# td-kwj-zp2023/webgpu-msm-twisted-edwards

Measured on AMD Instinct MI355X. Metric: MSMs/sec at n=2^20 Twisted-Edwards BLS12 (pipelined throughput = 1000/ms_per_step; single-MSM latency in latency_ms), higher is better.
Workload: dtype u32

## Files before the change

webgpu-msm-twisted-edwards_amd/csrc/kernels.hip.hpp:

```cpp
#pragma once
#include <hip/hip_runtime.h>
#include "curve.hpp"

namespace te {

#define TE_BATCH_MAX 8
struct batch_ptrs { const uint4* p[TE_BATCH_MAX]; };
struct batch_slabs { uint32_t s[TE_BATCH_MAX]; };

struct digits_params {
  uint32_t half[10];
  uint32_t zero_digit;
  uint32_t sc_stride;
  uint32_t n, nst;
  int num_windows;
  int w_first, w_step, nw_local;
  uint32_t half_code, logS, P, CH, chunk_len;
};

struct pnt_slot { uint4 q[8]; };
__device__ __forceinline__ void prep_points_block(uint32_t blk, uint4* __restrict__ lds, const uint4* __restrict__ pts, pnt_slot* __restrict__ recs, uint32_t n) {
  const uint32_t t = threadIdx.x, base = blk * 256u;
  const bool active = t < 256u;
  const uint32_t pieces_in = (n - base < 256u ? n - base : 256u) * 4u;
// ... 530 lines not shown
  __syncthreads();
  const uint32_t c0 = cnt_s[t];
  const size_t gb = (size_t)k * g.B + (size_t)p * g.S + t;
  if (!single) {
    if (c0) atomicAdd(&a.bucket_count[gb], c0);
    wait_own_accesses();
    __syncthreads();
    if (t == 0) pj[2] = (handoff_arrive(&a.part_ticket[k * g.P + p]) + 1u == (cntp + TE_L2_CAP - 1u) / TE_L2_CAP) ? 1u : 0u;
    __syncthreads();
    if (pj[2]) (void)seg_plan_block(p, k, t < g.S ? ld_agent(a.bucket_count + gb) : 0u, g, a.pa, PL, pb, cntp, sbp);
    return;
  }
  if (t < g.S) a.bucket_count[gb] = c0;
  const uint32_t ex = seg_plan_block(p, k, c0, g, a.pa, PL, pb, cntp, sbp);
  if (t < g.S) a.pa.bucket_cursor[gb] = pb + ex + c0;
  off_s[t] = ex;
  __syncthreads();
#pragma unroll
  for (int c = 0; c < 5; c++) {
    uint32_t kv[8], iv[8]; piece_group<PK>(r, c, kv, iv);
    const uint32_t e0 = ((uint32_t)c * 256u + t) * 8u;
#pragma unroll
    for (int e = 0; e < 8; e++) {
      const uint32_t pos = e0 + (uint32_t)e;
      if (pos >= head && pos < total) list[atomicAdd(&off_s[kv[e] & 0x7fffu], 1u)] = iv[e] | ((kv[e] >> 15) << 31);
    }
  }
  __syncthreads();
  uint32_t* out = a.sorted + (size_t)k * g.n + pb;
  for (uint32_t s = t; s < cntp; s += 256u) out[s] = list[s];
}

#define TE_ORDER_REGS 32u
__device__ __forceinline__ void order_scatter_block(uint32_t ob, uint32_t nob, uint32_t* __restrict__ lds, const uint32_t* __restrict__ lenv, uint32_t ids,
                                                    const uint32_t* __restrict__ size_hist, uint32_t* __restrict__ rel_cursor,
                                                    uint32_t* __restrict__ order, uint32_t* __restrict__ num_segments, uint32_t max_len) {
  uint32_t* const h = lds; uint32_t* const base = lds + 1024; uint32_t* const sm = lds + 2048;
  const uint32_t per = (ids + nob - 1) / nob;
  const uint32_t lo = min(ids, ob * per), hi = min(ids, lo + per);
  const bool in_regs = per <= TE_ORDER_REGS * 256u;
  uint32_t lv[TE_ORDER_REGS];
  if (in_regs) {
#pragma unroll
    for (uint32_t j = 0; j < TE_ORDER_REGS; j++) { const uint32_t g = lo + j * 256u + threadIdx.x; lv[j] = g < hi ? lenv[g] : TE_SEG_INVALID; }
  }
  for (uint32_t j = threadIdx.x; j < 1024u; j += 256u) h[j] = 0;
  {
    uint32_t run = 0;
    for (uint32_t c = (1023u - min(max_len, 1023u)) >> 8; c < 4u; c++) {
      const uint32_t s = 1023u - (c * 256u + threadIdx.x);
      uint32_t part[TE_HIST_COPIES];
#pragma unroll
      for (uint32_t r = 0; r < TE_HIST_COPIES; r++) part[r] = size_hist[r * 1024u + s];
      uint32_t cnt_s = 0;
#pragma unroll
      for (uint32_t r = 0; r < TE_HIST_COPIES; r++) cnt_s += part[r];
      uint32_t bt;
      const uint32_t ex = block_excl_scan(cnt_s, sm, bt);
      base[s] = run + ex;
      run += bt;
    }
    if (ob == 0 && threadIdx.x == 0) *num_segments = run;
  }
  __syncthreads();
  if (in_regs) {
#pragma unroll
    for (uint32_t j = 0; j < TE_ORDER_REGS; j++) if (lv[j] != TE_SEG_INVALID) atomicAdd(&h[min(lv[j], 1023u)], 1u);
  } else {
    for (uint32_t g = lo + threadIdx.x; g < hi; g += 256u) { const uint32_t l = lenv[g]; if (l != TE_SEG_INVALID) atomicAdd(&h[min(l, 1023u)], 1u); }
  }
  __syncthreads();
  for (uint32_t j = threadIdx.x; j < 1024u; j += 256u) { base[j] += h[j] ? atomicAdd(&rel_cursor[j], h[j]) : 0u; h[j] = 0; }
  __syncthreads();
  if (in_regs) {
#pragma unroll
    for (uint32_t j = 0; j < TE_ORDER_REGS; j++) {
      if (lv[j] == TE_SEG_INVALID) continue;
      const uint32_t sz = min(lv[j], 1023u);
      order[base[sz] + atomicAdd(&h[sz], 1u)] = lo + j * 256u + threadIdx.x;
    }
  } else {
    for (uint32_t g = lo + threadIdx.x; g < hi; g += 256u) {
      const uint32_t l = lenv[g];
      if (l == TE_SEG_INVALID) continue;
      const uint32_t sz = min(l, 1023u);
      order[base[sz] + atomicAdd(&h[sz], 1u)] = g;
    }
  }
}

#define TE_PLACE_LDS_WORDS (4u * 256u + TE_L2_LIST + TE_L2_LIST / 4u + 2u + 17u)
template <bool PK>
__device__ __forceinline__ void l2_place_piece(uint32_t p, uint32_t k, uint32_t a0, uint32_t b0, uint32_t* __restrict__ lds,
                                               const uint16_t* __restrict__ part_keys, const uint32_t* __restrict__ part_idx,
                                               uint32_t* __restrict__ bucket_cursor, uint32_t* __restrict__ sorted, const sort_geom& g) {
  uint32_t* const cnt_s = lds; uint32_t* const lex_s = lds + 256; uint32_t* const off_s = lds + 512; uint32_t* const gbase_s = lds + 768;
  uint32_t* const list = lds + 1024;
  uint8_t* const list_b = reinterpret_cast<uint8_t*>(list + TE_L2_LIST);
  uint32_t* const sm = list + TE_L2_LIST + TE_L2_LIST / 4u + 2u;
  const uint32_t t = threadIdx.x, len = b0 - a0;
  const uint16_t* keys_row = part_keys + (size_t)k * g.nst; const uint32_t* idx_row = part_idx + (size_t)k * g.nst;
  uint32_t* out = sorted + (size_t)k * g.n;
  cnt_s[t] = 0u;
  __syncthreads();
  piece_regs r; uint32_t head, total;
  load_piece<PK>(keys_row, idx_row, a0, b0, t, true, r, head, total);
#pragma unroll
  for (int c = 0; c < 5; c++) {
    uint32_t kv[8], iv[8]; piece_group<PK>(r, c, kv, iv);
    const uint32_t e0 = ((uint32_t)c * 256u + t) * 8u;
#pragma unroll
    for (int e = 0; e < 8; e++) { const uint32_t pos = e0 + (uint32_t)e; if (pos >= head && pos < total) atomicAdd(&cnt_s[kv[e] & 0x7fffu], 1u); }
  }
  __syncthreads();
  wave0_excl_scan(cnt_s, lex_s, 256u, &sm[16]);
  {
    const uint32_t c0 = cnt_s[t];
    gbase_s[t] = c0 ? atomicAdd(&bucket_cursor[(size_t)k * g.B + (size_t)p * g.S + t], c0) : 0u;
  }
  __syncthreads();
  off_s[t] = lex_s[t];
  gbase_s[t] -= lex_s[t];
  __syncthreads();
#pragma unroll
  for (int c = 0; c < 5; c++) {
    uint32_t kv[8], iv[8]; piece_group<PK>(r, c, kv, iv);
    const uint32_t e0 = ((uint32_t)c * 256u + t) * 8u;
#pragma unroll
    for (int e = 0; e < 8; e++) {
      const uint32_t pos = e0 + (uint32_t)e;
      if (pos >= head && pos < total) {
        const uint32_t b = kv[e] & 0x7fffu;
        const uint32_t slot = atomicAdd(&off_s[b], 1u);
        list[slot] = iv[e] | ((kv[e] >> 15) << 31); list_b[slot] = (uint8_t)b;
      }
    }
  }
  __syncthreads();
  for (uint32_t s = t; s < len; s += 256u) out[gbase_s[list_b[s]] + s] = list[s];
}

struct order_args { const uint32_t* lenv; uint32_t ids; const uint32_t* size_hist; uint32_t* rel_cursor; uint32_t* order; uint32_t* num_segments; uint32_t order_cols, max_len; };
template <bool PK>
__global__ void __launch_bounds__(256, TE_L2_WAVES) k_l2_place_order(const uint16_t* __restrict__ part_keys, const uint32_t* __restrict__ part_idx,
                                                           const uint32_t* __restrict__ part_start, const uint32_t* __restrict__ part_count,
                                                           uint32_t* __restrict__ bucket_cursor, uint32_t* __restrict__ sorted, sort_geom g, order_args oa) {
  __shared__ uint32_t lds[TE_PLACE_LDS_WORDS];
  if (blockIdx.x < oa.order_cols) {
    order_scatter_block(blockIdx.y * oa.order_cols + blockIdx.x, gridDim.y * oa.order_cols, lds, oa.lenv, oa.ids, oa.size_hist, oa.rel_cursor, oa.order, oa.num_segments, oa.max_len);
    return;
  }
  const uint32_t k = gridDim.y - 1u - blockIdx.y;
  const uint32_t px = blockIdx.x - oa.order_cols, extra = gridDim.x - oa.order_cols - g.P, bx = px < extra ? g.P + px : px - extra;
  const uint32_t* pc = part_count + k * g.P;
  uint32_t p, j;
  if (!l2_piece_of_block(bx, pc, g.P, bx < g.P ? 0u : part_count[gridDim.y * g.P + k], lds, lds + 32, p, j)) return;
  const uint32_t cntp = pc[p], pb = part_start[k * g.P + p];
  if (cntp <= TE_L2_CAP) return;
  const uint32_t a0 = pb + j * TE_L2_CAP;
  l2_place_piece<PK>(p, k, a0, min(pb + cntp, a0 + TE_L2_CAP), lds, part_keys, part_idx, bucket_cursor, sorted, g);
}

template <int N> struct geo {
  static constexpr uint32_t PW = 4u * N;
  static constexpr uint32_t PQ = PW / 4u;
  static constexpr uint32_t RW = N == 9 ? 27u : 4u * N;
  static constexpr uint32_t SQ = N == 9 ? 8u : N;
  static constexpr uint32_t LQ = (RW + 3u) / 4u;
};
template <int N> struct rec_slot { uint4 q[geo<N>::SQ]; };
static_assert(sizeof(rec_slot<9>) == sizeof(pnt_slot) && sizeof(rec_slot<14>) == 224, "record slots");

template <int N> __device__ __forceinline__ pnt_t<N> load_pnt(const rec_slot<N>* __restrict__ recs, uint32_t entry) {
  const uint4* q = recs[entry & 0x7fffffffu].q;
  constexpr uint32_t LQ = geo<N>::LQ;
  uint4 u[LQ];
#pragma unroll
  for (uint32_t j = 0; j < LQ; j++) u[j] = q[j];
  uint32_t w[4 * LQ];
#pragma unroll
  for (uint32_t j = 0; j < LQ; j++) { w[4 * j] = u[j].x; w[4 * j + 1] = u[j].y; w[4 * j + 2] = u[j].z; w[4 * j + 3] = u[j].w; }
  pnt_t<N> r;
// ... 50 lines not shown
  uint32_t w[42];
#pragma unroll
  for (int j = 0; j < 10; j++) { w[4 * j] = u[j].v[0]; w[4 * j + 1] = u[j].v[1]; w[4 * j + 2] = u[j].v[2]; w[4 * j + 3] = u[j].v[3]; }
  w[40] = t.v[0]; w[41] = t.v[1];
  pnt_aff377 r;
#pragma unroll
  for (int j = 0; j < 14; j++) { r.hm.v[j] = w[j]; r.hp.v[j] = w[14 + j]; r.dt.v[j] = w[28 + j]; }
  return r;
}
__device__ __forceinline__ void store_pnt_aff377(rec_aff377* dst, const pnt_aff377& r) {
#pragma unroll
  for (int j = 0; j < 14; j++) { dst->w[j] = r.hm.v[j]; dst->w[14 + j] = r.hp.v[j]; dst->w[28 + j] = r.dt.v[j]; }
}
template <int N, int RK> struct rec_kind;
template <int N> struct rec_kind<N, 0> {
  using slot = rec_slot<N>; using pnt = pnt_t<N>;
  static __device__ __forceinline__ pnt load(const slot* __restrict__ recs, uint32_t e) { return load_pnt<N>(recs, e); }
};
template <> struct rec_kind<14, 1> {
  using slot = rec_aff377; using pnt = pnt_aff377;
  static __device__ __forceinline__ pnt load(const slot* __restrict__ recs, uint32_t e) { return load_pnt_aff377(recs, e); }
};

struct __attribute__((aligned(4))) idx4 { uint32_t v[4]; };
#define TE_CLK_SLOTS 64u
#define TE_IDX_STRIP 16u
template <int N, int RK = 0>
__global__ void __launch_bounds__(256, N == 9 ? 3 : 2) k_accumulate(const typename rec_kind<N, RK>::slot* __restrict__ recs, const uint32_t* __restrict__ sorted,
                                                    const uint32_t* __restrict__ bucket_start, const uint32_t* __restrict__ bucket_count,
                                                    const uint32_t* __restrict__ seg_base, const uint32_t* __restrict__ seg_bucket,
                                                    const uint32_t* __restrict__ seg_lenv, const uint32_t* __restrict__ order,
                                                    const uint32_t* __restrict__ num_segments, ete_t<N>* __restrict__ buckets,
                                                    ete_t<N>* __restrict__ seg_out, uint32_t n, uint32_t logB, uint32_t seg_len, uint32_t ids, uint32_t onto,
                                                    uint32_t win_per_msm, batch_slabs slabs, unsigned long long* __restrict__ clk) {
  __shared__ uint32_t idx_strip[256 * TE_IDX_STRIP];
  using RT = rec_kind<N, RK>; using P = typename RT::pnt;
#if defined(TE_ACC_TWO_WAVES)
  if constexpr (N == 9) asm volatile("" ::: "v175");
#endif
  unsigned long long* const slot = clk ? clk + (blockIdx.x & (TE_CLK_SLOTS - 1u)) : nullptr;
  const unsigned long long t0_wall = clk ? (unsigned long long)wall_clock64() : 0ull, t0_core = clk ? (unsigned long long)clock64() : 0ull;
  if (clk && threadIdx.x == 0) atomicMax(slot, ~t0_wall);
  const uint32_t gid = blockIdx.x * 256u + threadIdx.x;
  if (gid >= (order ? *num_segments : ids)) return;
  const uint32_t sgm = order ? order[gid] : gid;
  const uint32_t g = seg_bucket[sgm];
  if (g == TE_SEG_INVALID) return;
  const uint32_t k = g >> logB;
  recs += (size_t)slabs.s[k / win_per_msm] * n;
  const uint32_t part = sgm - seg_base[g];
  const uint32_t cnt = seg_lenv[sgm];
  const uint32_t* lst = sorted + (size_t)k * n + bucket_start[g] + part * seg_len;
  ete_t<N> acc = (onto && part == 0u) ? load_ete<N>(buckets + g) : ete_identity_t<N>();
  if (cnt) {
    const uint32_t last = cnt - 1u;
    uint32_t j0 = 0;
    uint32_t e = lst[0], e_n = lst[min(1u, last)];
    P cur = RT::load(recs, e);
    if (!(onto && part == 0u)) {
      const P first = pnt_cneg(cur, (e >> 31) != 0u);
      e = e_n; e_n = lst[min(2u, last)];
      cur = RT::load(recs, e);
      acc = ete_from_pnt(first);
      j0 = 1;
    }
    uint32_t* const strip = idx_strip + threadIdx.x * TE_IDX_STRIP;
    auto refill = [&](uint32_t pos) {
      const idx4* src = reinterpret_cast<const idx4*>(lst + pos);
      idx4* dst = reinterpret_cast<idx4*>(strip);
#pragma unroll
      for (uint32_t h = 0; h < TE_IDX_STRIP / 4u; h += 2u) {
        const idx4 v0 = src[h], v1 = src[h + 1u];
        dst[h] = v0; dst[h + 1u] = v1;
      }
    };
    if (((j0 + 2u) & (TE_IDX_STRIP - 1u)) != 0u) refill((j0 + 2u) & ~(TE_IDX_STRIP - 1u));
    for (uint32_t j = j0; j < cnt; j++) {
      const uint32_t e_cur = e;
      P nxt = cur;
      const uint32_t pn = j + 2u;
      if ((pn & (TE_IDX_STRIP - 1u)) == 0u) refill(pn);
      const uint32_t e_nn = strip[pn & (TE_IDX_STRIP - 1u)];
      if (j + 1 < cnt) { e = e_n; nxt = RT::load(recs, e); }
      acc = ete_madd(acc, pnt_cneg(cur, (e_cur >> 31) != 0u));
      cur = nxt; e_n = e_nn;
    }
  }
  const bool whole = bucket_count[g] <= seg_len;
  store_ete<N>(whole ? buckets + g : seg_out + sgm, acc);
  if (clk && (uint32_t)__lane_id() == (uint32_t)__ffsll((long long)__ballot(1)) - 1u) {
    const unsigned long long t1_wall = (unsigned long long)wall_clock64(), t1_core = (unsigned long long)clock64();
    atomicMax(slot + TE_CLK_SLOTS, t1_wall);
    atomicAdd(slot + 2u * TE_CLK_SLOTS, t1_core - t0_core); atomicAdd(slot + 3u * TE_CLK_SLOTS, t1_wall - t0_wall);
  }
}

template <int N> struct sum_job_t {
  const ete_t<N>* in; ete_t<N>* out;
  uint32_t n_out;
  uint32_t K, inner;
  uint32_t in_per_window, out_per_window;
};
template <int N> struct sum_jobs_t { sum_job_t<N> j[4]; };
template <int N> __device__ __forceinline__ ete_t<N> pair_swap(const ete_t<N>& a) {
  ete_t<N> r;
#pragma unroll
  for (int i = 0; i < N; i++) {
    r.x.v[i] = (uint32_t)__builtin_amdgcn_mov_dpp((int)a.x.v[i], 0xb1, 0xf, 0xf, true);
    r.y.v[i] = (uint32_t)__builtin_amdgcn_mov_dpp((int)a.y.v[i], 0xb1, 0xf, 0xf, true);
    r.z.v[i] = (uint32_t)__builtin_amdgcn_mov_dpp((int)a.z.v[i], 0xb1, 0xf, 0xf, true);
    r.t.v[i] = (uint32_t)__builtin_amdgcn_mov_dpp((int)a.t.v[i], 0xb1, 0xf, 0xf, true);
  }
  return r;
}
template <int N, bool PAIR>
__global__ void __launch_bounds__(256, N == 9 ? 2 : 1) k_sum_groups(sum_jobs_t<N> js, uint32_t nw) {
  const sum_job_t<N>& j = js.j[blockIdx.y];
  constexpr uint32_t TPO = PAIR ? 2u : 1u;
  const uint32_t total = j.n_out * nw * TPO, Kt = j.K / TPO;
  for (uint32_t gt = blockIdx.x * 256u + threadIdx.x; gt < total; gt += gridDim.x * 256u) {
    const uint32_t g = gt / TPO, half = gt % TPO;
// ... 512 lines not shown
```

webgpu-msm-twisted-edwards_amd/csrc/te_msm.hip:

```cpp
#include <hip/hip_runtime.h>
#include <stdint.h>
#include <stdio.h>
#include <stdlib.h>
#include <string.h>
#include <string>
#include <vector>
#include <deque>
#include <algorithm>
#include <functional>
#include <chrono>
#include <thread>
#include <mutex>
#include <condition_variable>
#include <memory>
#if defined(__x86_64__)
#include <immintrin.h>
#endif

#include "../../include/te_msm.h"
#include "host_tail.hpp"
#include "synth.hpp"
#include "kernels.hip.hpp"
#include "check.hip.hpp"
#include "from_x.hip.hpp"
// ... 18 lines not shown
                                            : curve_sizes{TE_MSM_POINT_BYTES, TE_MSM_SCALAR_BYTES, sizeof(te::ete), sizeof(te::rec_slot<9>), TE_MSM_PARTIAL_BYTES, 64};
}
inline size_t rec_bytes_of(int curve, int rec_kind) { return (curve == TE_MSM_CURVE_BLS12_377_G1 && rec_kind == 1) ? sizeof(te::rec_aff377) : sizes_of(curve).rec; }
static_assert(TE377_TAIL_ROW_BYTES == TE_MSM_PARTIAL_BYTES_BLS12_377 && sizeof(te::ete_t<14>) * 5 == TE377_TAIL_ROW_BYTES, "row layout");
constexpr size_t TE_MAX_ROW_BYTES = TE377_TAIL_ROW_BYTES;

struct plan_t {
  int curve = 0;
  int c = 0, W = 0, nw = 0;
  int nw1 = 0, batch = 1;
  int w_first = 0, w_step = 1;
  uint32_t B = 0, logB = 0;
  int signed_digits = 1;
  uint32_t dw[4] = {0, 0, 0, 0};
  uint32_t CH = 0, chunk_len = 0, nst = 0;
  uint32_t seg_len = 64;
  uint32_t S = 0, logS = 0, P = 0;
  uint32_t packed = 0;
  int rec_kind = 0;
  int fb_rb = 0, fb_c = 0, fb_W = 0;
};

struct workset_t {
  hipStream_t stream = nullptr, copy_stream = nullptr;
  int hw_queue_class = -1;
  hipEvent_t ev_copy = nullptr, ev_start = nullptr;
  size_t cap[40] = {};
  uint8_t* d_recs = nullptr;
  uint16_t *d_digits = nullptr, *d_part_keys = nullptr;
  uint32_t *d_counts1 = nullptr, *d_part_start = nullptr, *d_part_count = nullptr, *d_part_idx = nullptr, *d_seg_part_base = nullptr;
  uint32_t *d_bucket_count = nullptr, *d_bucket_start = nullptr, *d_bucket_cursor = nullptr, *d_sorted = nullptr;
  uint32_t *d_seg_base = nullptr, *d_seg_bucket = nullptr, *d_seg_lenv = nullptr, *d_order = nullptr;
  uint32_t *d_split_list = nullptr, *d_chunk_list = nullptr;
  uint8_t *d_seg_out = nullptr, *d_buckets = nullptr, *d_red[4] = {};
  uint32_t *d_zero = nullptr; size_t zero_words = 0;
  size_t zero_clean_words = 0;
  uint32_t *d_err = nullptr, *d_num_seg = nullptr, *d_size_hist = nullptr, *d_size_cursor = nullptr;
  uint32_t* d_part_ticket = nullptr;
  uint8_t* d_partials = nullptr;
  uint32_t* h_err = nullptr;
  uint8_t* h_partials = nullptr;
  uint32_t* h_err_dev = nullptr;
  bool rows_on_host = false;
  hipEvent_t ev_done = nullptr;
  hipEvent_t ev_result = nullptr;
  hipEvent_t ev[ST_COUNT + 1] = {};
  plan_t plan; uint64_t n = 0; bool used = false;
  te_sched::slot_t slot;
  std::string job_err;
  int prof_level = 0;
  hipStream_t last_stream = nullptr;
  void *d_in_points = nullptr, *d_in_scalars = nullptr; size_t cap_in_points = 0, cap_in_scalars = 0;
  std::vector<hipEvent_t> piece_events;
  uint8_t* h_ring = nullptr; std::vector<hipEvent_t> ring_ev; size_t ring_next = 0;
  uint64_t idle_calls = 0;
  uint32_t* d_fb_remap = nullptr;
  uint32_t* d_fb_fill = nullptr;
  const void* fb_scalars = nullptr; uint64_t fb_n = 0;
  int slab = -1;
  bool slab_run = false;
  const uint8_t* recs_last = nullptr;
  te_bases* bound = nullptr;
  int pt_rc = 0; int64_t pt_index = -1; int pt_reason = 0;
  uint8_t* d_batch_rows = nullptr;
  uint32_t* d_in_idx = nullptr;
};
// ... 132 lines not shown
  p.nw1 = p.nw; p.batch = batch; p.nw *= batch;
  p.logB = (uint32_t)(p.signed_digits ? p.c - 1 : p.c); p.B = 1u << p.logB;
  for (int k = 0; k < 4; k++) p.dw[k] = (p.logB + 3u - (uint32_t)k) / 4u;
#ifndef TE_SCATTER_BLOCKS
#define TE_SCATTER_BLOCKS 1024u
#endif
  uint32_t ch = p.nw > 0 ? TE_SCATTER_BLOCKS / (uint32_t)p.nw : 1u;
  if (ch < 1) ch = 1;
  if (ch > 256) ch = 256;
#ifndef TE_SCATTER_MINCHUNK
#define TE_SCATTER_MINCHUNK 4096u
#endif
  const uint32_t by_n = (uint32_t)((n + TE_SCATTER_MINCHUNK - 1) / TE_SCATTER_MINCHUNK);
  if (ch > by_n) ch = by_n ? by_n : 1;
  p.nst = (uint32_t)((n + 7) & ~(uint64_t)7);
  p.chunk_len = (uint32_t)((p.nst + ch - 1) / ch);
  p.chunk_len = (p.chunk_len + 4095u) & ~4095u;
  ch = (p.nst + p.chunk_len - 1) / p.chunk_len;
  p.CH = ch;
  p.S = p.B < 256u ? p.B : 256u;
  if (force_seg) {
    p.seg_len = force_seg;
  } else if (ctx->opt_seg_len) {
    p.seg_len = (uint32_t)ctx->opt_seg_len;
  } else {
    uint64_t a = (2 * n + p.B - 1) / p.B, s2 = 16;
    while (s2 < a && s2 < 64) s2 <<= 1;
    p.seg_len = (uint32_t)s2;
  }
  p.P = p.B / p.S; p.logS = ilog2(p.S);
  p.packed = (ctx->opt_packed && n <= (1ull << 23)) ? 1u : 0u;
}

template <typename T> int ensure(te_ctx* ctx, workset_t& ws, T*& ptr, size_t& cap_bytes, size_t need_elems) {
  const size_t need = need_elems * sizeof(T);
  if (ptr && need <= cap_bytes) return 0;
  if (ptr) HIP_TRY(ctx, hipFree(ptr));
  ptr = nullptr; cap_bytes = 0;
  HIP_TRY(ctx, hipMalloc((void**)&ptr, need ? need : 16));
  cap_bytes = need;
  return 0;
}

int ensure_buffers(te_ctx* ctx, gpu_t& d, workset_t& ws, uint64_t n, const plan_t& p, bool need_recs = true) {
  HIP_TRY(ctx, hipSetDevice(d.device));
  const size_t nd = (size_t)p.nw * p.nst + 64, wb = (size_t)p.nw * p.B, ab = sizes_of(p.curve).acc;
  int rc = 0;
  if (need_recs && (rc = ensure(ctx, ws, ws.d_recs, ws.cap[0], (size_t)n * sizes_of(p.curve).rec * (size_t)p.batch))) return rc;
  if ((rc = ensure(ctx, ws, ws.d_digits, ws.cap[1], nd))) return rc;
  if ((rc = ensure(ctx, ws, ws.d_sorted, ws.cap[2], nd))) return rc;
  {
    const size_t c1 = (size_t)p.nw * p.CH * p.P;
    ws.zero_words = Z_END + c1 + wb + (size_t)p.nw * p.P + 64;
    { const uint32_t* before = ws.d_zero; if ((rc = ensure(ctx, ws, ws.d_zero, ws.cap[3], ws.zero_words))) return rc; if (ws.d_zero != before) ws.zero_clean_words = 0; }
    ws.d_err = ws.d_zero; ws.d_num_seg = ws.d_zero + Z_KEEP; ws.d_size_hist = ws.d_zero + Z_HIST; ws.d_size_cursor = ws.d_zero + Z_CURSOR;
    ws.d_partials = reinterpret_cast<uint8_t*>(ws.d_zero + Z_ROWS);
    ws.d_counts1 = ws.d_zero + Z_END; ws.d_bucket_count = ws.d_counts1 + c1; ws.d_part_ticket = ws.d_bucket_count + wb;
    ws.d_fb_fill = ws.d_part_ticket + (size_t)p.nw * p.P;
  }
  if (p.fb_rb && (rc = ensure(ctx, ws, ws.d_fb_remap, ws.cap[27], nd))) return rc;
  if ((rc = ensure(ctx, ws, ws.d_bucket_start, ws.cap[5], wb))) return rc;
  if ((rc = ensure(ctx, ws, ws.d_bucket_cursor, ws.cap[16], wb))) return rc;
  if ((rc = ensure(ctx, ws, ws.d_seg_part_base, ws.cap[17], (size_t)p.nw * p.P))) return rc;
  const size_t smax = wb + (size_t)p.nw * (n / (uint64_t)p.seg_len) + 16;
  if ((rc = ensure(ctx, ws, ws.d_order, ws.cap[7], smax))) return rc;
  if ((rc = ensure(ctx, ws, ws.d_seg_bucket, ws.cap[20], smax))) return rc;
  if ((rc = ensure(ctx, ws, ws.d_seg_lenv, ws.cap[21], smax))) return rc;
  if ((rc = ensure(ctx, ws, ws.d_seg_out, ws.cap[22], smax * ab))) return rc;
  if ((rc = ensure(ctx, ws, ws.d_seg_base, ws.cap[23], wb + 1))) return rc;
  if ((rc = ensure(ctx, ws, ws.d_split_list, ws.cap[24], wb + 1))) return rc;
  if ((rc = ensure(ctx, ws, ws.d_chunk_list, ws.cap[26], 2 * (wb + smax / TE_GIANT_RUN + 2)))) return rc;
  if ((rc = ensure(ctx, ws, ws.d_part_start, ws.cap[6], (size_t)p.nw * p.P))) return rc;
  if ((rc = ensure(ctx, ws, ws.d_buckets, ws.cap[8], wb * ab))) return rc;
  if ((rc = ensure(ctx, ws, ws.d_part_count, ws.cap[9], (size_t)p.nw * p.P + (size_t)p.nw))) return rc;
  if ((rc = ensure(ctx, ws, ws.d_part_keys, ws.cap[14], p.packed ? 8 : nd))) return rc;
  if ((rc = ensure(ctx, ws, ws.d_part_idx, ws.cap[15], nd))) return rc;
  if ((rc = ensure(ctx, ws, ws.d_red[0], ws.cap[10], (wb / 2 + 1) * ab))) return rc;
  if ((rc = ensure(ctx, ws, ws.d_red[1], ws.cap[11], (wb / 4 + 1) * ab))) return rc;
  if ((rc = ensure(ctx, ws, ws.d_red[2], ws.cap[12], (wb / 2 + 1) * ab))) return rc;
  if ((rc = ensure(ctx, ws, ws.d_red[3], ws.cap[13], (wb / 4 + 1) * ab))) return rc;
  return 0;
}

template <int C> void launch_digits(const te::batch_ptrs& sc, int batch, uint16_t* dg, const te::digits_params& prm, uint32_t* err, uint32_t* counts1, hipStream_t s) {
  hipLaunchKernelGGL(te::k_digits<C>, dim3((prm.nst + TE_DIG_BLOCK - 1u) / TE_DIG_BLOCK, batch), dim3(TE_DIG_THREADS), 0, s, sc, dg, prm, err, counts1);
}
static_assert(TE_BATCH_MAX == TE_MSM_MAX_BATCH, "batch tables");
template <int C> void launch_digits_ragged(const void* sc, const te::ragged_tab& tab, int batch, uint16_t* dg, const te::digits_params& prm, uint32_t* err, uint32_t* counts1, hipStream_t s) {
  hipLaunchKernelGGL(te::k_digits_ragged<C>, dim3((prm.nst + TE_DIG_BLOCK - 1u) / TE_DIG_BLOCK, batch), dim3(TE_DIG_THREADS), 0, s, static_cast<const uint4*>(sc), tab, dg, prm, err, counts1);
}
static_assert(TE_RAGGED_MAX == TE_BATCH_SEQ_MAX && TE_BATCH_SEQ_MAX == TE_MSM_BATCH_SEQ_MAX, "ragged tables");

struct msm_launch {
  te_ctx* ctx; workset_t& ws; plan_t p;
  const void* d_points; const void* d_scalars; uint64_t n; void* d_partials_out;
  int prof;
  hipStream_t stream;
  bool own_rows = false;
  bool onto = false;
  bool host_rows = false;
  uint8_t* recs_rw = nullptr;
  uint8_t* recs_out() const { return recs_rw ? recs_rw : ws.d_recs; }
  bool have_recs = false;
  void count_conversion() const { __atomic_fetch_add(&ctx->stat_record_conversions, (int64_t)1, __ATOMIC_RELAXED); }
  const uint32_t* fb_remap = nullptr;
  const uint8_t* bound = nullptr;
  const te::ragged_tab* ragged = nullptr;
  const uint32_t* idx = nullptr; uint32_t idx_count = 0, idx_pos = 0;
  static bool rows_to_host(const te_ctx* ctx, const gpu_t& d, const plan_t& p, bool own_rows) {
    return own_rows && p.nw > 0 && p.batch == 1 && p.w_first == 0 && p.w_step == 1 && ctx->opt_prezero;
  }
  uint32_t n32() const { return (uint32_t)n; }
  uint32_t total() const { return (uint32_t)p.nw * p.B; }
  uint32_t smax() const { return total() + (uint32_t)((uint64_t)p.nw * (n / p.seg_len)); }
  uint32_t chunk_cap() const { return total() + smax() / TE_GIANT_RUN + 2u; }
  const void* points_of(int m) const { return p.batch > 1 ? static_cast<const void* const*>(d_points)[m] : d_points; }
  const void* scalars_of(int m) const { return p.batch > 1 ? static_cast<const void* const*>(d_scalars)[m] : d_scalars; }
  void mark(int i) const { if (prof >= 2 || (prof == 1 && (i == ST_ACCUM || i == ST_ACCUM + 1))) (void)hipEventRecord(ws.ev[i], stream); }

  bool can_fuse_conversion() const { return prof < 2 && p.nw > 0; }
  int front() {
    if (have_recs) return front_scalars();
    if (can_fuse_conversion()) return front_scalars(true);
    if (int rc = front_scalars()) return rc;
    return front_points();
  }

  int prep_rows(te::batch_ptrs& tab, te::batch_slabs& row_slab) const {
    const te::batch_slabs sl = slabs();
    memset(&tab, 0, sizeof tab); memset(&row_slab, 0, sizeof row_slab);
    int rows = 0;
    for (int m = 0; m < p.batch; m++) if ((int)sl.s[m] == m) { tab.p[rows] = (const uint4*)points_of(m); row_slab.s[rows] = (uint32_t)m; rows++; }
    return rows;
  }

  te::batch_slabs slabs() const {
    te::batch_slabs r; memset(&r, 0, sizeof r);
    for (int m = 0; m < p.batch; m++) {
      int first = m;
      for (int j = 0; j < m; j++) if (points_of(j) == points_of(m)) { first = j; break; }
      r.s[m] = (uint32_t)first;
    }
    return r;
  }

  int front_points() {
    const uint32_t n32 = this->n32();
    mark(ST_PREP);
// ... 73 lines not shown
          const uint32_t per_row = (n32 + 511u) / 512u;
          hipLaunchKernelGGL(te::k_part_scatter_prep377, dim3(sblocks + rows * per_row), dim3(512), 0, stream, sa, sblocks, tab, row_slab,
                             reinterpret_cast<te::rec_slot<14>*>(recs_out()), n32, per_row, rows * per_row);
        } else {
          const uint32_t per_row = (n32 + 255u) / 256u;
          hipLaunchKernelGGL(te::k_part_scatter_prep, dim3(sblocks + rows * per_row), dim3(512), 0, stream, sa, sblocks, tab, row_slab,
                             reinterpret_cast<te::pnt_slot*>(recs_out()), n32, per_row, rows * per_row);
        }
      } else if (idx) {
        hipLaunchKernelGGL(te::k_part_scatter_indexed, dim3(p.CH, p.nw), dim3(512), 0, stream, sa, te::index_args{idx, idx_count, idx_pos, ws.d_err});
      } else {
        hipLaunchKernelGGL(te::k_part_scatter, dim3(p.CH, p.nw), dim3(512), 0, stream, sa);
      }
    }
    mark(ST_BSORT);
    if (p.nw > 0) {
      const uint32_t l2_blocks = p.P + n32 / TE_L2_CAP + 1u;
      te::l2_args la;
      la.part_keys = ws.d_part_keys; la.part_idx = ws.d_part_idx; la.part_start = ws.d_part_start; la.part_count = ws.d_part_count;
      la.bucket_count = ws.d_bucket_count; la.sorted = ws.d_sorted; la.part_ticket = ws.d_part_ticket; la.g = sg;
      la.pa.part_start = ws.d_part_start; la.pa.part_count = ws.d_part_count; la.pa.seg_part_base = ws.d_seg_part_base;
      la.pa.bucket_start = ws.d_bucket_start; la.pa.bucket_cursor = ws.d_bucket_cursor; la.pa.seg_base = ws.d_seg_base; la.pa.seg_bucket = ws.d_seg_bucket;
      la.pa.seg_lenv = ws.d_seg_lenv; la.pa.size_hist = ws.d_size_hist; la.pa.split_list = ws.d_split_list; la.pa.split_count = ws.d_num_seg + 1;
      la.pa.chunk_list = ws.d_chunk_list; la.pa.seg_len = p.seg_len; la.pa.cap_w = cap_w; la.pa.chunk_cap = chunk_cap();
      if (p.packed) hipLaunchKernelGGL(te::k_l2_local<true>, dim3(l2_blocks, p.nw), dim3(256), 0, stream, la);
      else hipLaunchKernelGGL(te::k_l2_local<false>, dim3(l2_blocks, p.nw), dim3(256), 0, stream, la);
      te::order_args oa;
      oa.lenv = ws.d_seg_lenv; oa.ids = smax(); oa.size_hist = ws.d_size_hist; oa.rel_cursor = ws.d_size_cursor; oa.order = ws.d_order; oa.num_segments = ws.d_num_seg;
      {
        const uint32_t by_regs = (smax() + TE_ORDER_REGS * 256u * (uint32_t)p.nw - 1u) / (TE_ORDER_REGS * 256u * (uint32_t)p.nw);
        oa.order_cols = std::min(64u, std::max(by_regs, (uint32_t)std::max(1, 128 / p.nw)));
      }
      oa.max_len = std::min(p.seg_len, 1023u);
      if (p.packed)
        hipLaunchKernelGGL(te::k_l2_place_order<true>, dim3(oa.order_cols + l2_blocks, p.nw), dim3(256), 0, stream, ws.d_part_keys, ws.d_part_idx, ws.d_part_start,
                           ws.d_part_count, ws.d_bucket_cursor, ws.d_sorted, sg, oa);
      else
        hipLaunchKernelGGL(te::k_l2_place_order<false>, dim3(oa.order_cols + l2_blocks, p.nw), dim3(256), 0, stream, ws.d_part_keys, ws.d_part_idx, ws.d_part_start,
                           ws.d_part_count, ws.d_bucket_cursor, ws.d_sorted, sg, oa);
    }
    mark(ST_ORDER);
    return 0;
  }

  bool bls() const { return p.curve == TE_MSM_CURVE_BLS12_377_G1; }

  template <int N, int RK> int accumulate_t() {
    mark(ST_ACCUM);
    if (p.nw > 0) {
      const uint32_t n32 = this->n32(), smax = this->smax();
      const uint32_t* order = ctx->opt_sort ? ws.d_order : nullptr;
      using slot_t = typename te::rec_kind<N, RK>::slot;
      hipLaunchKernelGGL((te::k_accumulate<N, RK>), dim3((smax + 255) / 256), dim3(256), 0, stream, reinterpret_cast<const slot_t*>(bound ? bound : recs_out()), ws.d_sorted,
                         ws.d_bucket_start, ws.d_bucket_count, ws.d_seg_base, ws.d_seg_bucket, ws.d_seg_lenv, order, ws.d_num_seg,
                         reinterpret_cast<te::ete_t<N>*>(ws.d_buckets), reinterpret_cast<te::ete_t<N>*>(ws.d_seg_out), n32, p.logB, p.seg_len, smax, onto ? 1u : 0u,
                         ragged ? (uint32_t)p.nw : (uint32_t)p.nw1, ragged ? te::batch_slabs{} : slabs(),
                         prof ? reinterpret_cast<unsigned long long*>(ws.d_zero + Z_CLOCK) : nullptr);
    }
    return 0;
  }
  int accumulate() { return bls() ? (p.rec_kind == 1 ? accumulate_t<14, 1>() : accumulate_t<14, 0>()) : accumulate_t<9, 0>(); }

  template <int N> int combine_t() {
    if (p.nw <= 0) return 0;
    using E = te::ete_t<N>;
    hipLaunchKernelGGL(te::k_seg_combine_all<N>, dim3(256 + 1024), dim3(256), 0, stream, ws.d_split_list, ws.d_num_seg + 1, ws.d_chunk_list,
                       ws.d_bucket_count, ws.d_seg_base, reinterpret_cast<E*>(ws.d_seg_out), reinterpret_cast<E*>(ws.d_buckets), p.seg_len, chunk_cap(), 256u,
                       ws.d_bucket_start, ws.d_bucket_cursor);
    return 0;
  }
  int combine() { return bls() ? combine_t<14>() : combine_t<9>(); }

  template <int N> int reduce_t() {
    if (p.nw > 0) {
      using E = te::ete_t<N>;
      const uint32_t w0 = p.dw[0], w1 = p.dw[1], w2 = p.dw[2], w3 = p.dw[3];
      const uint32_t L = 1u << (w0 + w1), H = 1u << (w2 + w3);
      struct chain_t { const E* cur; uint32_t n, r; E* buf[2]; int pp; };
      E* const bk = reinterpret_cast<E*>(ws.d_buckets);
      chain_t ch[2] = {{bk, p.B, L, {reinterpret_cast<E*>(ws.d_red[0]), reinterpret_cast<E*>(ws.d_red[1])}, 0},
                       {bk, p.B, H, {reinterpret_cast<E*>(ws.d_red[2]), reinterpret_cast<E*>(ws.d_red[3])}, 0}};
      for (;;) {
        te::sum_jobs_t<N> js; memset(&js, 0, sizeof js);
        uint32_t most = 0; int nj = 0;
        for (int i = 0; i < 2; i++) {
          chain_t& c = ch[i];
          if (c.r <= 4u) continue;
          const uint32_t K = (c.r % 8u == 0) ? 8u : (c.r % 4u == 0) ? 4u : 2u;
          te::sum_job_t<N>& j = js.j[nj++];
          j.in = c.cur; j.out = c.buf[c.pp]; j.K = K; j.n_out = c.n / K;
// ... 302 lines not shown
  HIP_TRY(ctx, hipEventRecord(ws.ev_done, stream));
  return 0;
}

int collect_stage_ms(te_ctx* ctx, const gpu_t& d, workset_t& ws) {
  if (!ws.prof_level) return 0;
  bool ok = true;
  for (int i = 0; i < ST_COUNT; i++) {
    float ms = -1.0f;
    if (ws.prof_level >= 2 || i == ST_ACCUM) ok = ok && hipEventElapsedTime(&ms, ws.ev[i], ws.ev[i + 1]) == hipSuccess;
    ctx->stage_ms[i] = ms;
  }
  {
    uint64_t raw[4 * TE_CLK_SLOTS]; memcpy(raw, ws.h_err + Z_CLOCK, sizeof raw);
    uint64_t c[4] = {0, 0, 0, 0};
    for (uint32_t i = 0; i < TE_CLK_SLOTS; i++) {
      c[0] = std::max(c[0], raw[i]); c[1] = std::max(c[1], raw[TE_CLK_SLOTS + i]);
      c[2] += raw[2 * TE_CLK_SLOTS + i]; c[3] += raw[3 * TE_CLK_SLOTS + i];
    }
    const int khz = d.wall_clock_khz;
    const bool have = c[0] && c[1] && khz > 0 && c[1] > ~c[0];
    const double ms = have ? (double)(c[1] - ~c[0]) / khz : -1.0;
    ctx->stage_ms[ST_COUNT] = (float)ms;
    ctx->stage_ms[ST_COUNT + 1] = (have && c[2] && c[3]) ? (float)((double)c[2] / (double)c[3] * khz * 1e-6) : -1.0f;
  }
  if (!ok) (void)hipGetLastError();
  ctx->have_stage_ms = ok;
  return 0;
}

void free_workset_buffers(workset_t& ws) {
  void** ptrs[] = {(void**)&ws.d_recs, (void**)&ws.d_digits, (void**)&ws.d_part_keys, (void**)&ws.d_zero, (void**)&ws.d_part_start, (void**)&ws.d_part_count,
                   (void**)&ws.d_part_idx, (void**)&ws.d_seg_part_base, (void**)&ws.d_bucket_start, (void**)&ws.d_bucket_cursor, (void**)&ws.d_sorted,
                   (void**)&ws.d_seg_base, (void**)&ws.d_seg_bucket, (void**)&ws.d_seg_lenv, (void**)&ws.d_order, (void**)&ws.d_split_list,
                   (void**)&ws.d_chunk_list, (void**)&ws.d_seg_out, (void**)&ws.d_buckets, (void**)&ws.d_red[0], (void**)&ws.d_red[1],
                   (void**)&ws.d_red[2], (void**)&ws.d_red[3], &ws.d_in_points, &ws.d_in_scalars, (void**)&ws.d_fb_remap, (void**)&ws.d_batch_rows, (void**)&ws.d_in_idx};
  for (void** q : ptrs) if (*q) { (void)hipFree(*q); *q = nullptr; }
  if (ws.h_ring) { (void)hipHostFree(ws.h_ring); ws.h_ring = nullptr; }
  memset(ws.cap, 0, sizeof ws.cap); ws.cap_in_points = ws.cap_in_scalars = 0;
  ws.zero_words = ws.zero_clean_words = 0;
  ws.d_err = ws.d_num_seg = ws.d_size_hist = ws.d_size_cursor = ws.d_counts1 = ws.d_bucket_count = ws.d_part_ticket = nullptr; ws.d_partials = nullptr;
  ws.used = false;
}

void free_dev(gpu_t& d) {
  (void)hipSetDevice(d.device);
  for (auto& sl : d.slabs) {
    if (sl.d) { (void)hipFree(sl.d); sl.d = nullptr; }
    for (hipEvent_t& e : sl.ev) if (e) { (void)hipEventDestroy(e); e = nullptr; }
    if (sl.conv_ev) { (void)hipEventDestroy(sl.conv_ev); sl.conv_ev = nullptr; }
  }
  d.slabs.clear();
  if (d.chk_stream) (void)hipStreamDestroy(d.chk_stream);
  if (d.chk_pts) (void)hipFree(d.chk_pts);
  if (d.chk_word) (void)hipFree(d.chk_word);
  if (d.chk_host) (void)hipHostFree(d.chk_host);
  d.chk_stream = nullptr; d.chk_pts = nullptr; d.chk_cap = 0; d.chk_word = d.chk_host = nullptr;
  if (d.h_batch_rows) (void)hipHostFree(d.h_batch_rows);
  d.h_batch_rows = nullptr; d.h_batch_cap = 0;
  for (workset_t& ws : d.ws) {
    free_workset_buffers(ws);
    if (ws.h_err) (void)hipHostFree(ws.h_err);
    for (hipEvent_t e : ws.ring_ev) if (e) (void)hipEventDestroy(e);
    if (ws.ev_done) (void)hipEventDestroy(ws.ev_done);
    if (ws.ev_result) (void)hipEventDestroy(ws.ev_result);
    for (auto& ev : ws.ev) if (ev) (void)hipEventDestroy(ev);
    if (ws.ev_copy) (void)hipEventDestroy(ws.ev_copy);
// ... 2239 lines not shown
  if (device_index < 0 || (size_t)device_index >= ctx->devs.size() || first > total || count > total - first) return set_err(ctx, TE_MSM_EINVAL, "bad arguments");
  if (record_bytes) *record_bytes = (int)bases->rec_bytes;
  uint64_t bytes = count * bases->rec_bytes;
  if (bytes > cap) bytes = cap;
  if (!bytes) return 0;
  HIP_TRY(ctx, hipSetDevice(ctx->devs[(size_t)device_index].device));
  HIP_TRY(ctx, hipMemcpy(dst, bases->recs[(size_t)device_index] + first * bases->rec_bytes, bytes, hipMemcpyDeviceToHost));
  return (int64_t)bytes;
}

int64_t te_msm_debug_read(te_ctx* ctx, const char* stage, void* dst, uint64_t cap) {
  device_guard restore_callers_device;
  if (!ctx || !stage || !dst) return TE_MSM_EINVAL;
  drain_workers(ctx);
  gpu_t& d = ctx->devs[0];
  workset_t& ws = d.ws[d.last_ws];
  if (!ws.used) return set_err(ctx, TE_MSM_ESTATE, "no run yet");
  const plan_t& p = ws.plan; const uint64_t n = ws.n;
  const void* src = nullptr; uint64_t bytes = 0;
  if (ws.zero_clean_words && (!strcmp(stage, "bucket_count") || !strcmp(stage, "num_segments") || !strcmp(stage, "partials")))
    return set_err(ctx, TE_MSM_ESTATE, "this stage lives in the block that is cleared behind an MSM's read-back: set option prezero = 0 before the run to keep it");
  if (!strcmp(stage, "records")) {
    if (!ws.recs_last) return set_err(ctx, TE_MSM_ESTATE, "the last run gathered from a bound point set: the work set holds no records of its own");
    src = ws.recs_last; bytes = n * sizes_of(p.curve).rec;
  }
  else if (!strcmp(stage, "digits")) { src = ws.d_digits; bytes = (uint64_t)p.nw * p.nst * 2; }
  else if (!strcmp(stage, "bucket_count")) { src = ws.d_bucket_count; bytes = (uint64_t)p.nw * p.B * 4; }
  else if (!strcmp(stage, "bucket_start")) { src = ws.d_bucket_start; bytes = (uint64_t)p.nw * p.B * 4; }
  else if (!strcmp(stage, "sorted")) { src = ws.d_sorted; bytes = (uint64_t)p.nw * n * 4; }
  else if (!strcmp(stage, "num_segments")) { src = ws.d_num_seg; bytes = 4; }
  else if (!strcmp(stage, "seg_bucket")) { src = ws.d_seg_bucket; bytes = ((uint64_t)p.nw * p.B + (uint64_t)p.nw * (n / p.seg_len)) * 4; }
  else if (!strcmp(stage, "seg_len")) { src = ws.d_seg_lenv; bytes = ((uint64_t)p.nw * p.B + (uint64_t)p.nw * (n / p.seg_len)) * 4; }
  else if (!strcmp(stage, "order")) { src = ws.d_order; bytes = ((uint64_t)p.nw * p.B + (uint64_t)p.nw * (n / p.seg_len)) * 4; }
  else if (!strcmp(stage, "part_start")) { src = ws.d_part_start; bytes = (uint64_t)p.nw * p.P * 4; }
  else if (!strcmp(stage, "part_count")) { src = ws.d_part_count; bytes = (uint64_t)p.nw * p.P * 4; }
  else if (!strcmp(stage, "part_keys") && !p.packed) { src = ws.d_part_keys; bytes = (uint64_t)p.nw * p.nst * 2; }
  else if (!strcmp(stage, "part_idx") && !p.packed) { src = ws.d_part_idx; bytes = (uint64_t)p.nw * p.nst * 4; }
  else if (!strcmp(stage, "part_keys") || !strcmp(stage, "part_idx")) {
    const bool want_keys = stage[5] == 'k';
    const uint64_t words = (uint64_t)p.nw * p.nst;
    std::vector<uint32_t> pk(words);
    HIP_TRY(ctx, hipSetDevice(d.device));
    HIP_TRY(ctx, hipDeviceSynchronize());
    HIP_TRY(ctx, hipMemcpy(pk.data(), ws.d_part_idx, words * 4, hipMemcpyDeviceToHost));
    uint64_t out_bytes = words * (want_keys ? 2 : 4);
    if (out_bytes > cap) out_bytes = cap;
    if (want_keys) { uint16_t* o = static_cast<uint16_t*>(dst); for (uint64_t i = 0; i < out_bytes / 2; i++) o[i] = (uint16_t)(((pk[i] >> 23) & 0xffu) | ((pk[i] >> 31) << 15)); }
    else { uint32_t* o = static_cast<uint32_t*>(dst); for (uint64_t i = 0; i < out_bytes / 4; i++) o[i] = pk[i] & 0x7fffffu; }
    return (int64_t)out_bytes;
  }
  else if (!strcmp(stage, "buckets")) { src = ws.d_buckets; bytes = (uint64_t)p.nw * p.B * sizes_of(p.curve).acc; }
  else if (!strcmp(stage, "partials")) { src = ws.d_partials; bytes = (uint64_t)p.W * sizes_of(p.curve).row; }
  else return set_err(ctx, TE_MSM_EINVAL, "unknown stage");
  if (bytes > cap) bytes = cap;
  HIP_TRY(ctx, hipSetDevice(d.device));
  HIP_TRY(ctx, hipDeviceSynchronize());
  HIP_TRY(ctx, hipMemcpy(dst, src, bytes, hipMemcpyDeviceToHost));
  return (int64_t)bytes;
}

}
```

Before: 1105.

## Precompute packed segment descriptors in order scatter for bucket accumulation

```diff
diff --git a/webgpu-msm-twisted-edwards_amd/csrc/kernels.hip.hpp b/webgpu-msm-twisted-edwards_amd/csrc/kernels.hip.hpp
--- a/webgpu-msm-twisted-edwards_amd/csrc/kernels.hip.hpp
+++ b/webgpu-msm-twisted-edwards_amd/csrc/kernels.hip.hpp
@@ -586,17 +586,34 @@
 }
 
 #define TE_ORDER_REGS 32u
+#define TE_SCHED_WHOLE (1u << 30)
+#define TE_SCHED_FIRST (1u << 31)
+#define TE_SCHED_CNT 0x3fffffffu
+struct sched_args {
+  uint4* sched;
+  const uint32_t *seg_bucket, *bucket_start, *seg_base, *bucket_count; uint32_t n, logB, seg_len;
+};
+__device__ __forceinline__ uint4 seg_descriptor(uint32_t sgm, uint32_t g, uint32_t cnt, uint32_t bstart, uint32_t sbase, uint32_t bcount, const sched_args& s) {
+  const uint32_t part = sgm - sbase;
+  return make_uint4((g >> s.logB) * s.n + bstart + part * s.seg_len, g, sgm,
+                    cnt | (bcount <= s.seg_len ? TE_SCHED_WHOLE : 0u) | (part == 0u ? TE_SCHED_FIRST : 0u));
+}
 __device__ __forceinline__ void order_scatter_block(uint32_t ob, uint32_t nob, uint32_t* __restrict__ lds, const uint32_t* __restrict__ lenv, uint32_t ids,
                                                     const uint32_t* __restrict__ size_hist, uint32_t* __restrict__ rel_cursor,
-                                                    uint32_t* __restrict__ order, uint32_t* __restrict__ num_segments, uint32_t max_len) {
+                                                    uint32_t* __restrict__ order, uint32_t* __restrict__ num_segments, uint32_t max_len, const sched_args& sa) {
   uint32_t* const h = lds; uint32_t* const base = lds + 1024; uint32_t* const sm = lds + 2048;
   const uint32_t per = (ids + nob - 1) / nob;
   const uint32_t lo = min(ids, ob * per), hi = min(ids, lo + per);
   const bool in_regs = per <= TE_ORDER_REGS * 256u;
-  uint32_t lv[TE_ORDER_REGS];
+  const bool descr = sa.sched != nullptr;
+  uint32_t lv[TE_ORDER_REGS], gv[TE_ORDER_REGS];
   if (in_regs) {
 #pragma unroll
     for (uint32_t j = 0; j < TE_ORDER_REGS; j++) { const uint32_t g = lo + j * 256u + threadIdx.x; lv[j] = g < hi ? lenv[g] : TE_SEG_INVALID; }
+    if (descr) {
+#pragma unroll
+      for (uint32_t j = 0; j < TE_ORDER_REGS; j++) { const uint32_t g = lo + j * 256u + threadIdx.x; gv[j] = g < hi ? sa.seg_bucket[g] : TE_SEG_INVALID; }
+    }
   }
   for (uint32_t j = threadIdx.x; j < 1024u; j += 256u) h[j] = 0;
   {
@@ -626,7 +643,26 @@
   __syncthreads();
   for (uint32_t j = threadIdx.x; j < 1024u; j += 256u) { base[j] += h[j] ? atomicAdd(&rel_cursor[j], h[j]) : 0u; h[j] = 0; }
   __syncthreads();
-  if (in_regs) {
+  if (in_regs && descr) {
+#pragma unroll
+    for (uint32_t j0 = 0; j0 < TE_ORDER_REGS; j0 += 8u) {
+      uint32_t bs[8], sb[8], bc[8];
+#pragma unroll
+      for (uint32_t u = 0; u < 8u; u++) {
+        const uint32_t g = lv[j0 + u] != TE_SEG_INVALID ? gv[j0 + u] : 0u;
+        bs[u] = sa.bucket_start[g]; sb[u] = sa.seg_base[g]; bc[u] = sa.bucket_count[g];
+      }
+#pragma unroll
+      for (uint32_t u = 0; u < 8u; u++) {
+        const uint32_t j = j0 + u;
+        if (lv[j] == TE_SEG_INVALID) continue;
+        const uint32_t sz = min(lv[j], 1023u), sgm = lo + j * 256u + threadIdx.x;
+        const uint32_t slot = base[sz] + atomicAdd(&h[sz], 1u);
+        order[slot] = sgm;
+        sa.sched[slot] = seg_descriptor(sgm, gv[j], lv[j], bs[u], sb[u], bc[u], sa);
+      }
+    }
+  } else if (in_regs) {
 #pragma unroll
     for (uint32_t j = 0; j < TE_ORDER_REGS; j++) {
       if (lv[j] == TE_SEG_INVALID) continue;
@@ -638,7 +674,9 @@
       const uint32_t l = lenv[g];
       if (l == TE_SEG_INVALID) continue;
       const uint32_t sz = min(l, 1023u);
-      order[base[sz] + atomicAdd(&h[sz], 1u)] = g;
+      const uint32_t slot = base[sz] + atomicAdd(&h[sz], 1u);
+      order[slot] = g;
+      if (descr) { const uint32_t b = sa.seg_bucket[g]; sa.sched[slot] = seg_descriptor(g, b, l, sa.bucket_start[b], sa.seg_base[b], sa.bucket_count[b], sa); }
     }
   }
 }
@@ -694,14 +732,14 @@
   for (uint32_t s = t; s < len; s += 256u) out[gbase_s[list_b[s]] + s] = list[s];
 }
 
-struct order_args { const uint32_t* lenv; uint32_t ids; const uint32_t* size_hist; uint32_t* rel_cursor; uint32_t* order; uint32_t* num_segments; uint32_t order_cols, max_len; };
+struct order_args { const uint32_t* lenv; uint32_t ids; const uint32_t* size_hist; uint32_t* rel_cursor; uint32_t* order; uint32_t* num_segments; uint32_t order_cols, max_len; sched_args sa; };
 template <bool PK>
 __global__ void __launch_bounds__(256, TE_L2_WAVES) k_l2_place_order(const uint16_t* __restrict__ part_keys, const uint32_t* __restrict__ part_idx,
                                                            const uint32_t* __restrict__ part_start, const uint32_t* __restrict__ part_count,
                                                            uint32_t* __restrict__ bucket_cursor, uint32_t* __restrict__ sorted, sort_geom g, order_args oa) {
   __shared__ uint32_t lds[TE_PLACE_LDS_WORDS];
   if (blockIdx.x < oa.order_cols) {
-    order_scatter_block(blockIdx.y * oa.order_cols + blockIdx.x, gridDim.y * oa.order_cols, lds, oa.lenv, oa.ids, oa.size_hist, oa.rel_cursor, oa.order, oa.num_segments, oa.max_len);
+    order_scatter_block(blockIdx.y * oa.order_cols + blockIdx.x, gridDim.y * oa.order_cols, lds, oa.lenv, oa.ids, oa.size_hist, oa.rel_cursor, oa.order, oa.num_segments, oa.max_len, oa.sa);
     return;
   }
   const uint32_t k = gridDim.y - 1u - blockIdx.y;
@@ -818,7 +856,8 @@
                                                     const uint32_t* __restrict__ seg_lenv, const uint32_t* __restrict__ order,
                                                     const uint32_t* __restrict__ num_segments, ete_t<N>* __restrict__ buckets,
                                                     ete_t<N>* __restrict__ seg_out, uint32_t n, uint32_t logB, uint32_t seg_len, uint32_t ids, uint32_t onto,
-                                                    uint32_t win_per_msm, batch_slabs slabs, unsigned long long* __restrict__ clk) {
+                                                    uint32_t win_per_msm, batch_slabs slabs, unsigned long long* __restrict__ clk,
+                                                    const uint4* __restrict__ sched) {
   __shared__ uint32_t idx_strip[256 * TE_IDX_STRIP];
   using RT = rec_kind<N, RK>; using P = typename RT::pnt;
 #if defined(TE_ACC_TWO_WAVES)
@@ -829,21 +868,31 @@
   if (clk && threadIdx.x == 0) atomicMax(slot, ~t0_wall);
   const uint32_t gid = blockIdx.x * 256u + threadIdx.x;
   if (gid >= (order ? *num_segments : ids)) return;
-  const uint32_t sgm = order ? order[gid] : gid;
-  const uint32_t g = seg_bucket[sgm];
-  if (g == TE_SEG_INVALID) return;
-  const uint32_t k = g >> logB;
+  uint32_t sgm, g, fl;
+  const uint32_t* lst;
+  if (sched) {
+    const uint4 d = sched[gid];
+    sgm = d.z; g = d.y; fl = d.w;
+    if (g == TE_SEG_INVALID) return;
+    lst = sorted + d.x;
+  } else {
+    sgm = order ? order[gid] : gid;
+    g = seg_bucket[sgm];
+    if (g == TE_SEG_INVALID) return;
+    const uint32_t part = sgm - seg_base[g];
+    fl = seg_lenv[sgm] | (part == 0u ? TE_SCHED_FIRST : 0u);
+    lst = sorted + (size_t)(g >> logB) * n + bucket_start[g] + part * seg_len;
+  }
+  const uint32_t k = g >> logB, cnt = fl & TE_SCHED_CNT;
+  const bool cont = onto && (fl & TE_SCHED_FIRST) != 0u;
   recs += (size_t)slabs.s[k / win_per_msm] * n;
-  const uint32_t part = sgm - seg_base[g];
-  const uint32_t cnt = seg_lenv[sgm];
-  const uint32_t* lst = sorted + (size_t)k * n + bucket_start[g] + part * seg_len;
-  ete_t<N> acc = (onto && part == 0u) ? load_ete<N>(buckets + g) : ete_identity_t<N>();
+  ete_t<N> acc = cont ? load_ete<N>(buckets + g) : ete_identity_t<N>();
   if (cnt) {
     const uint32_t last = cnt - 1u;
     uint32_t j0 = 0;
     uint32_t e = lst[0], e_n = lst[min(1u, last)];
     P cur = RT::load(recs, e);
-    if (!(onto && part == 0u)) {
+    if (!cont) {
       const P first = pnt_cneg(cur, (e >> 31) != 0u);
       e = e_n; e_n = lst[min(2u, last)];
       cur = RT::load(recs, e);
@@ -872,7 +921,7 @@
       cur = nxt; e_n = e_nn;
     }
   }
-  const bool whole = bucket_count[g] <= seg_len;
+  const bool whole = sched ? (fl & TE_SCHED_WHOLE) != 0u : bucket_count[g] <= seg_len;
   store_ete<N>(whole ? buckets + g : seg_out + sgm, acc);
   if (clk && (uint32_t)__lane_id() == (uint32_t)__ffsll((long long)__ballot(1)) - 1u) {
     const unsigned long long t1_wall = (unsigned long long)wall_clock64(), t1_core = (unsigned long long)clock64();
diff --git a/webgpu-msm-twisted-edwards_amd/csrc/te_msm.hip b/webgpu-msm-twisted-edwards_amd/csrc/te_msm.hip
--- a/webgpu-msm-twisted-edwards_amd/csrc/te_msm.hip
+++ b/webgpu-msm-twisted-edwards_amd/csrc/te_msm.hip
@@ -74,6 +74,7 @@
   uint32_t *d_bucket_count = nullptr, *d_bucket_start = nullptr, *d_bucket_cursor = nullptr, *d_sorted = nullptr;
   uint32_t *d_seg_base = nullptr, *d_seg_bucket = nullptr, *d_seg_lenv = nullptr, *d_order = nullptr;
   uint32_t *d_split_list = nullptr, *d_chunk_list = nullptr;
+  uint4* d_sched = nullptr;
   uint8_t *d_seg_out = nullptr, *d_buckets = nullptr, *d_red[4] = {};
   uint32_t *d_zero = nullptr; size_t zero_words = 0;
   size_t zero_clean_words = 0;
@@ -272,6 +273,8 @@
   p.packed = (ctx->opt_packed && n <= (1ull << 23)) ? 1u : 0u;
 }
 
+bool sched_fits(const plan_t& p, uint64_t n) { return (uint64_t)p.nw * n + 64 < (1ull << 32); }
+
 template <typename T> int ensure(te_ctx* ctx, workset_t& ws, T*& ptr, size_t& cap_bytes, size_t need_elems) {
   const size_t need = need_elems * sizeof(T);
   if (ptr && need <= cap_bytes) return 0;
@@ -304,6 +307,7 @@
   if ((rc = ensure(ctx, ws, ws.d_seg_part_base, ws.cap[17], (size_t)p.nw * p.P))) return rc;
   const size_t smax = wb + (size_t)p.nw * (n / (uint64_t)p.seg_len) + 16;
   if ((rc = ensure(ctx, ws, ws.d_order, ws.cap[7], smax))) return rc;
+  if (sched_fits(p, n) && (rc = ensure(ctx, ws, ws.d_sched, ws.cap[30], smax))) return rc;
   if ((rc = ensure(ctx, ws, ws.d_seg_bucket, ws.cap[20], smax))) return rc;
   if ((rc = ensure(ctx, ws, ws.d_seg_lenv, ws.cap[21], smax))) return rc;
   if ((rc = ensure(ctx, ws, ws.d_seg_out, ws.cap[22], smax * ab))) return rc;
@@ -354,6 +358,7 @@
   uint32_t total() const { return (uint32_t)p.nw * p.B; }
   uint32_t smax() const { return total() + (uint32_t)((uint64_t)p.nw * (n / p.seg_len)); }
   uint32_t chunk_cap() const { return total() + smax() / TE_GIANT_RUN + 2u; }
+  uint4* sched() const { return ctx->opt_sort && sched_fits(p, n) && ws.cap[30] >= (size_t)smax() * sizeof(uint4) ? ws.d_sched : nullptr; }
   const void* points_of(int m) const { return p.batch > 1 ? static_cast<const void* const*>(d_points)[m] : d_points; }
   const void* scalars_of(int m) const { return p.batch > 1 ? static_cast<const void* const*>(d_scalars)[m] : d_scalars; }
   void mark(int i) const { if (prof >= 2 || (prof == 1 && (i == ST_ACCUM || i == ST_ACCUM + 1))) (void)hipEventRecord(ws.ev[i], stream); }
@@ -493,6 +498,8 @@
         oa.order_cols = std::min(64u, std::max(by_regs, (uint32_t)std::max(1, 128 / p.nw)));
       }
       oa.max_len = std::min(p.seg_len, 1023u);
+      oa.sa.sched = sched(); oa.sa.seg_bucket = ws.d_seg_bucket; oa.sa.bucket_start = ws.d_bucket_start; oa.sa.seg_base = ws.d_seg_base;
+      oa.sa.bucket_count = ws.d_bucket_count; oa.sa.n = n32; oa.sa.logB = p.logB; oa.sa.seg_len = p.seg_len;
       if (p.packed)
         hipLaunchKernelGGL(te::k_l2_place_order<true>, dim3(oa.order_cols + l2_blocks, p.nw), dim3(256), 0, stream, ws.d_part_keys, ws.d_part_idx, ws.d_part_start,
                            ws.d_part_count, ws.d_bucket_cursor, ws.d_sorted, sg, oa);
@@ -516,7 +523,7 @@
                          ws.d_bucket_start, ws.d_bucket_count, ws.d_seg_base, ws.d_seg_bucket, ws.d_seg_lenv, order, ws.d_num_seg,
                          reinterpret_cast<te::ete_t<N>*>(ws.d_buckets), reinterpret_cast<te::ete_t<N>*>(ws.d_seg_out), n32, p.logB, p.seg_len, smax, onto ? 1u : 0u,
                          ragged ? (uint32_t)p.nw : (uint32_t)p.nw1, ragged ? te::batch_slabs{} : slabs(),
-                         prof ? reinterpret_cast<unsigned long long*>(ws.d_zero + Z_CLOCK) : nullptr);
+                         prof ? reinterpret_cast<unsigned long long*>(ws.d_zero + Z_CLOCK) : nullptr, sched());
     }
     return 0;
   }
@@ -885,7 +892,7 @@
 void free_workset_buffers(workset_t& ws) {
   void** ptrs[] = {(void**)&ws.d_recs, (void**)&ws.d_digits, (void**)&ws.d_part_keys, (void**)&ws.d_zero, (void**)&ws.d_part_start, (void**)&ws.d_part_count,
                    (void**)&ws.d_part_idx, (void**)&ws.d_seg_part_base, (void**)&ws.d_bucket_start, (void**)&ws.d_bucket_cursor, (void**)&ws.d_sorted,
-                   (void**)&ws.d_seg_base, (void**)&ws.d_seg_bucket, (void**)&ws.d_seg_lenv, (void**)&ws.d_order, (void**)&ws.d_split_list,
+                   (void**)&ws.d_seg_base, (void**)&ws.d_seg_bucket, (void**)&ws.d_seg_lenv, (void**)&ws.d_order, (void**)&ws.d_sched, (void**)&ws.d_split_list,
                    (void**)&ws.d_chunk_list, (void**)&ws.d_seg_out, (void**)&ws.d_buckets, (void**)&ws.d_red[0], (void**)&ws.d_red[1],
                    (void**)&ws.d_red[2], (void**)&ws.d_red[3], &ws.d_in_points, &ws.d_in_scalars, (void**)&ws.d_fb_remap, (void**)&ws.d_batch_rows, (void**)&ws.d_in_idx};
   for (void** q : ptrs) if (*q) { (void)hipFree(*q); *q = nullptr; }
@@ -3191,6 +3198,11 @@
   else if (!strcmp(stage, "seg_bucket")) { src = ws.d_seg_bucket; bytes = ((uint64_t)p.nw * p.B + (uint64_t)p.nw * (n / p.seg_len)) * 4; }
   else if (!strcmp(stage, "seg_len")) { src = ws.d_seg_lenv; bytes = ((uint64_t)p.nw * p.B + (uint64_t)p.nw * (n / p.seg_len)) * 4; }
   else if (!strcmp(stage, "order")) { src = ws.d_order; bytes = ((uint64_t)p.nw * p.B + (uint64_t)p.nw * (n / p.seg_len)) * 4; }
+  else if (!strcmp(stage, "sched")) {
+    if (!ws.d_sched || !ctx->opt_sort || !sched_fits(p, n) || ws.cap[30] < ((uint64_t)p.nw * p.B + (uint64_t)p.nw * (n / p.seg_len)) * 16) return set_err(ctx, TE_MSM_ESTATE, "the last run wrote no segment descriptors");
+    src = ws.d_sched; bytes = ((uint64_t)p.nw * p.B + (uint64_t)p.nw * (n / p.seg_len)) * 16;
+  }
+  else if (!strcmp(stage, "seg_base")) { src = ws.d_seg_base; bytes = (uint64_t)p.nw * p.B * 4; }
   else if (!strcmp(stage, "part_start")) { src = ws.d_part_start; bytes = (uint64_t)p.nw * p.P * 4; }
   else if (!strcmp(stage, "part_count")) { src = ws.d_part_count; bytes = (uint64_t)p.nw * p.P * 4; }
   else if (!strcmp(stage, "part_keys") && !p.packed) { src = ws.d_part_keys; bytes = (uint64_t)p.nw * p.nst * 2; }
```

After: 1098. No clear change (-0.6%).
